# liuyuan-pal/Gen6D

Hardware: NVIDIA H100
Metric: poses/sec end-to-end (128^2 crop, 64 refs, 3 refine iters) (higher is better)
Workload: dtype f32

## Files before the change

### gen6d_b200/_lib.py

```python
import ctypes as C
import os
import re

HERE = os.path.dirname(os.path.abspath(__file__))
LIB_PATH = os.path.join(HERE, 'libgen6d_b200.so')
HEADER_PATH = os.path.join(os.path.dirname(HERE), 'include', 'gen6d_b200.h')

G6D_DET_MAX_SCALES = 8
G6D_GLUE_MAX_OBJECTS = 16
G6D_DET_MAX_INSTANCES = 16
G6D_DET_MAX_PEAK_RADIUS = 3
G6D_DET_MAX_BOXES = 256
G6D_ATTENTION_MAX_SMEM_FLOATS = 12288 - 32
G6D_FRAMES_MAX = 1024
G6D_FRAME_RGB, G6D_FRAME_NV12 = 0, 1
G6D_DRAW_MAX_BOXES = 16
PRO_NONE, PRO_AFFINE, PRO_AFFINE_RELU, PRO_CORR = 0, 1, 2, 3
ACT_NONE, ACT_RELU, ACT_LEAKY01 = 0, 1, 2
TC_TF32, TC_F16 = 0, 1
TC_PRENORM, TC_REUSE_IM2COL, TC_FOLD_SPLITS = 1, 4, 32


class ConvDesc(C.Structure):
    _fields_ = [(n, C.c_int) for n in ('B', 'D', 'H', 'W', 'Cin', 'in_cstride', 'in_coff', 'Cout', 'kd', 'kh', 'kw',
# ... 100 lines not shown
    'g6d_conv_tc_workspace_bytes_ex': [C.POINTER(ConvDesc), I, I],
    'g6d_conv_tc_ex': [C.POINTER(ConvDesc), P, P, P, I, I, P, P, P, P, P, P, L, I, P],
    'g6d_pack_conv_weight_tc': [P, P, P, I, I, I, I, I, P, I, P],
    'g6d_split_operand': [P, P, P, L, I, P],
    'g6d_transpose2d': [P, P, I, I, P],
    'g6d_linear_smallm': [P, P, P, P, I, I, I, I, P],
    'g6d_det_score_fuse': [C.POINTER(DetMaps), I, P, P, P, P, P, P],
    'g6d_det_parse': [P, P, P, I, I, I, I, P, P, P],
    'g6d_det_parse_peaks': [P, P, P, I, I, I, I, I, I, F, F, F, P, P, P, P, P],
    'g6d_det_parse_peaks_host': [P, P, P, I, I, I, I, I, I, F, F, F, P, P, P, P],
    'g6d_det_from_boxes': [P, P, I, I, I, F, P, P, P, P],
    'g6d_det_from_boxes_host': [P, P, I, I, I, F, P, P, P],
    'g6d_det_corr_rowsum': [P, P, I, I, I, I, I, P],
    'g6d_det_corr_rowsum_objects': [P, P, I, I, I, I, I, I, P],
    'g6d_sel_ref_sums': [P, I, I, I, P, P, P],
    'g6d_sel_corr_prologue': [P, P, P, I, I, I, F, P, P, P],
    'g6d_sel_corr_score': [P, P, I, I, I, P, P],
    'g6d_sel_corr_score3': [P, P, P, P, P, P, I, I, I, I, I, P, P, P, P],
    'g6d_sel_corr_score3_workspace_bytes': [I, I, I, I],
    'g6d_sel_vp_norm': [P, I, I, F, P, I, I, P],
    'g6d_sel_max_angle_add': [P, P, P, I, I, I, P],
    'g6d_attention': [P, P, P, P, I, I, I, P],
    'g6d_attention_headmajor': [P, P, P, P, I, I, I, P],
    'g6d_layernorm': [P, P, P, P, I, I, F, P],
    'g6d_sel_parse': [P, P, I, I, P, P, P],
    'g6d_ref_volume_fill': [P, P, P, P, P, P, I, I, I, I, I, I, I, I, P, P, P],
    'g6d_ref_pose_heads': [P, P, P, P, I, I, P],
    'g6d_pose_errors_workspace_bytes': [I, I],
    'g6d_pose_errors': [P, I, P, P, P, I, I, P, P, P],
}
_RESTYPE = {'g6d_pose_errors_workspace_bytes': L, 'g6d_sel_corr_score3_workspace_bytes': L, 'g6d_conv_workspace_bytes': L, 'g6d_conv_tc_workspace_bytes': L, 'g6d_conv_tc_workspace_bytes_ex': L, 'g6d_launch_count': L, 'g6d_last_error': C.c_char_p}

_lib = None


class Gen6DLibraryError(RuntimeError):
    pass

# ... 37 lines not shown
```

### gen6d_b200/csrc/selector.cu

```cuda
#include "common.cuh"

namespace g6d {

template <int C>
__global__ void __launch_bounds__(256) sel_corr_score_kernel(const float* __restrict__ ref,
                                                             const float* __restrict__ q, int S, int P,
                                                             float* __restrict__ score) {
    constexpr int V = C / 128;
    extern __shared__ float t_sh[];
    const int warp = threadIdx.x >> 5, lane = threadIdx.x & 31;
    const int nwarp = blockDim.x >> 5;
    __shared__ float s_red[8];
    for (int s = blockIdx.x; s < S; s += gridDim.x) {
        const float4* rs = reinterpret_cast<const float4*>(ref + (long long)s * P * C);
        float mx = -INFINITY;
        for (int p = warp; p < P; p += nwarp) {
            const float4* rp = rs + (long long)p * (C / 4);
            const float4* qp = reinterpret_cast<const float4*>(q + (long long)p * C);
            float4 rv[V];
#pragma unroll
            for (int i = 0; i < V; ++i) rv[i] = ldg_stream(rp + lane + 32 * i);
            float t = 0.f;
#pragma unroll
            for (int i = 0; i < V; ++i) {
// ... 15 lines not shown
        if (lane == 0) s_red[warp] = acc;
        __syncthreads();
        if (threadIdx.x == 0) {
            float a = 0.f;
            for (int w = 0; w < nwarp; ++w) a += s_red[w];
            score[s] = a;
        }
        __syncthreads();
    }
}

struct ScoreLevels {
    const float* ref[3];
    const float* q[3];
    int P[3];
    int S;
    long long row_end[3];
};

template <int C>
__device__ __forceinline__ float row_dot(const float4* __restrict__ rp, const float4* __restrict__ qp, int lane) {
    constexpr int V = C / 128;
    float4 rv[V];
#pragma unroll
    for (int i = 0; i < V; ++i) rv[i] = ldg_stream(rp + lane + 32 * i);
    float t = 0.f;
#pragma unroll
    for (int i = 0; i < V; ++i) {
        const float4 qv = __ldg(qp + lane + 32 * i);
        t = fmaf(rv[i].x, qv.x, fmaf(rv[i].y, qv.y, fmaf(rv[i].z, qv.z, fmaf(rv[i].w, qv.w, t))));
    }
    return t;
}

template <int C, bool FUSED>
__global__ void __launch_bounds__(256, 6) sel_corr_dots_kernel(const ScoreLevels L, float* __restrict__ t_out,
                                                            int* __restrict__ done, float* __restrict__ score,
                                                            long long chunk) {
    const int lane = threadIdx.x & 31, wib = threadIdx.x >> 5;
    const long long rows = L.row_end[2];
    auto locate = [&](long long row, const float4*& rp, const float4*& qp, int& item, int& P, long long& first) {
        const bool l0 = row < L.row_end[0], l1 = row < L.row_end[1];
        const long long lbase = l0 ? 0 : (l1 ? L.row_end[0] : L.row_end[1]);
        const long long local = row - lbase;
        P = l0 ? L.P[0] : (l1 ? L.P[1] : L.P[2]);
        const float* ref = l0 ? L.ref[0] : (l1 ? L.ref[1] : L.ref[2]);
        const float* q = l0 ? L.q[0] : (l1 ? L.q[1] : L.q[2]);
        const int sl = (int)(local / P);
        const int p = (int)(local - (long long)sl * P);
        item = (l0 ? 0 : (l1 ? 1 : 2)) * L.S + sl;
        first = lbase + (long long)sl * P;
        rp = reinterpret_cast<const float4*>(ref + local * C);
        qp = reinterpret_cast<const float4*>(q + (long long)p * C);
    };
    long long begin, end, stride;
    if (FUSED) {
        begin = (long long)blockIdx.x * chunk;
        end = min(rows, begin + chunk);
        stride = 16;
    } else {
        begin = 0; end = rows;
        stride = (((long long)gridDim.x * blockDim.x) >> 5) * 2;
    }
    const long long w0 = FUSED ? wib : (((long long)blockIdx.x * blockDim.x + threadIdx.x) >> 5);
    for (long long row = begin + w0 * 2; row < end; row += stride) {
        const float4 *r0, *q0, *r1, *q1;
        int item, P;
        long long first;
        locate(row, r0, q0, item, P, first);
        const bool two = row + 1 < end;
        locate(two ? row + 1 : row, r1, q1, item, P, first);
        float t0 = row_dot<C>(r0, q0, lane);
        float t1 = row_dot<C>(r1, q1, lane);
        t0 = warp_sum(t0);
        t1 = warp_sum(t1);
        if (lane == 0) {
            t_out[row] = t0;
            if (two) t_out[row + 1] = t1;
        }
    }
    if (!FUSED) return;
    if (lane == 0) __threadfence();
    __syncthreads();
    int n = 0;
    for (long long r = begin; r < end; ++n) {
        const float4 *rp, *qp;
        int item, P;
        long long first;
        locate(r, rp, qp, item, P, first);
        const long long next = min(end, first + P);
        if ((n & 7) == wib) {
            int last = 0;
            if (lane == 0) last = atomicAdd(done + item, (int)(next - r)) + (int)(next - r) == P;
            last = __shfl_sync(0xffffffffu, last, 0);
            if (last) {
                if (lane == 0) done[item] = 0;
                __threadfence();
                const float* tp = t_out + first;
                float m = -INFINITY;
                for (int p = lane; p < P; p += 32) m = fmaxf(m, __ldcg(tp + p));
                m = warp_max(m);
                float acc = 0.f;
                for (int p = lane; p < P; p += 32) { const float v = __ldcg(tp + p); acc += v * (v / m); }
                acc = warp_sum(acc);
                if (lane == 0) score[item] = acc;
            }
        }
        r = next;
    }
}

__global__ void sel_corr_finish_kernel(const ScoreLevels L, const float* __restrict__ t, float* __restrict__ score) {
    const int lane = threadIdx.x & 31;
    const int item = (int)(((long long)blockIdx.x * blockDim.x + threadIdx.x) >> 5);
    if (item >= 3 * L.S) return;
    const int l = item / L.S, s = item % L.S;
    const int P = l == 0 ? L.P[0] : (l == 1 ? L.P[1] : L.P[2]);
    const float* tp = t + (l == 0 ? 0 : (l == 1 ? L.row_end[0] : L.row_end[1])) + (long long)s * P;
    float m = -INFINITY;
    for (int p = lane; p < P; p += 32) m = fmaxf(m, tp[p]);
    m = warp_max(m);
    float acc = 0.f;
    for (int p = lane; p < P; p += 32) { const float v = tp[p]; acc += v * (v / m); }
    acc = warp_sum(acc);
    if (lane == 0) score[item] = acc;
}

__global__ void sel_ref_sums_kernel(const float* __restrict__ ref, int S, long long PC, int s_chunk,
                                    double* __restrict__ sum1, double* __restrict__ sum2) {
    const long long i = (long long)blockIdx.x * blockDim.x + threadIdx.x;
    if (i >= PC) return;
    const int s0 = blockIdx.y * s_chunk, s1 = min(S, s0 + s_chunk);
    double a = 0.0, b = 0.0;
    for (int s = s0; s < s1; ++s) {
        const double v = (double)ref[(long long)s * PC + i];
        a += v; b += v * v;
    }
    atomicAdd(sum1 + i, a);
    atomicAdd(sum2 + i, b);
}

__global__ void sel_corr_prologue_kernel(const float* __restrict__ q, const double* __restrict__ sum1,
                                         const double* __restrict__ sum2, int S, int P, int C, float eps,
                                         float* __restrict__ scale, float* __restrict__ shift) {
    const int c = blockIdx.x * 32 + (threadIdx.x & 31);
    const int row = threadIdx.x >> 5, nrow = blockDim.x >> 5;
    __shared__ double sm[8][32], sv[8][32];
    __shared__ float s_rstd[32];
    double m = 0.0, e2 = 0.0;
    if (c < C) {
        for (int p = row; p < P; p += nrow) {
            const double qv = (double)q[(long long)p * C + c];
            m += qv * sum1[(long long)p * C + c];
            e2 += qv * qv * sum2[(long long)p * C + c];
        }
    }
    sm[row][threadIdx.x & 31] = m; sv[row][threadIdx.x & 31] = e2;
    __syncthreads();
    if (row == 0 && c < C) {
// ... 3 lines not shown
        double var = e2 / n - mean * mean;
        var = var < 0.0 ? 0.0 : var;
        const double rstd = 1.0 / sqrt(var + (double)eps);
        s_rstd[threadIdx.x] = (float)rstd;
        shift[c] = (float)(-mean * rstd);
    }
    __syncthreads();
    if (c < C) {
        const float r = s_rstd[threadIdx.x & 31];
        for (int p = row; p < P; p += nrow) scale[(long long)p * C + c] = q[(long long)p * C + c] * r;
    }
}

__global__ void sel_vp_norm_kernel(const float* __restrict__ score, int n, float eps, float* __restrict__ feats,
                                   int cstride, int coff) {
    const int l = blockIdx.x;
    const float* s = score + (long long)l * n;
    __shared__ double r1[32], r2[32];
    double a = 0.0, b = 0.0;
    for (int i = threadIdx.x; i < n; i += blockDim.x) { const double v = s[i]; a += v; b += v * v; }
    a = warp_sum(a); b = warp_sum(b);
    if ((threadIdx.x & 31) == 0) { r1[threadIdx.x >> 5] = a; r2[threadIdx.x >> 5] = b; }
    __syncthreads();
    a = 0.0; b = 0.0;
    for (int w = 0; w < (int)(blockDim.x >> 5); ++w) { a += r1[w]; b += r2[w]; }
    const double mean = a / n;
    double var = b / n - mean * mean;
    var = var < 0.0 ? 0.0 : var;
    const float rstd = (float)(1.0 / sqrt(var + (double)eps));
    const float fm = (float)mean;
    for (int i = threadIdx.x; i < n; i += blockDim.x) feats[(long long)i * cstride + coff + l] = (s[i] - fm) * rstd;
    if (l == 0)
        for (int c = coff + (int)gridDim.x; c < cstride; ++c)
            for (int i = threadIdx.x; i < n; i += blockDim.x) feats[(long long)i * cstride + c] = 0.f;
}

__global__ void sel_max_angle_add_kernel(const float* __restrict__ x, const float* __restrict__ embed,
                                         float* __restrict__ out, int rfn, int an, int C) {
    const long long i = (long long)blockIdx.x * blockDim.x + threadIdx.x;
    if (i >= (long long)rfn * C) return;
    const int c = (int)(i % C);
    const int r = (int)(i / C);
    float m = -INFINITY;
    for (int a = 0; a < an; ++a) m = fmaxf(m, x[((long long)r * an + a) * C + c]);
    out[i] = m + embed[i];
}

__global__ void attention_kernel(const float* __restrict__ q, const float* __restrict__ k, const float* __restrict__ v,
                                 float* __restrict__ out, int n, int C, int heads) {
    extern __shared__ float sh[];
    const int i = blockIdx.x, h = blockIdx.y;
    const int D = C / heads;
    float* prob = sh;
// ... 22 lines not shown
    if ((threadIdx.x & 31) == 0) red[threadIdx.x >> 5] = sum;
    __syncthreads();
    sum = 0.f;
    for (int w = 0; w < (int)(blockDim.x >> 5); ++w) sum += red[w];
    for (int d = threadIdx.x; d < D; d += blockDim.x) {
        float acc = 0.f;
        for (int j = 0; j < n; ++j) acc = fmaf(prob[j], v[(long long)j * C + d * heads + h], acc);
        out[(long long)i * C + d * heads + h] = acc / sum;
    }
}

constexpr int ATT_TQ = 8, ATT_TK = 32, ATT_D = 64;
__global__ void __launch_bounds__(128) attention_hm_kernel(const float* __restrict__ q, const float* __restrict__ k,
                                                           const float* __restrict__ v, float* __restrict__ out, int n, int C) {
    extern __shared__ float sh[];
    const int npad = (n + 31) & ~31;
    float* qs = sh;
    float* kt = qs + ATT_TQ * ATT_D;
    float* sc = kt + ATT_TK * (ATT_D + 1);
    __shared__ float s_sum[ATT_TQ];
    const int t = threadIdx.x, lane = t & 31, warp = t >> 5;
    const int i0 = blockIdx.x * ATT_TQ, h = blockIdx.y;
    const float inv = rsqrtf((float)ATT_D);
    for (int e = t; e < ATT_TQ * ATT_D; e += 128) {
        const int qi = e / ATT_D, d = e % ATT_D;
        qs[e] = i0 + qi < n ? q[(long long)(i0 + qi) * C + h * ATT_D + d] : 0.f;
    }
    for (int j0 = 0; j0 < n; j0 += ATT_TK) {
        __syncthreads();
        for (int e = t; e < ATT_TK * ATT_D / 4; e += 128) {
// ... 90 lines not shown
extern "C" int g6d_sel_corr_score(const float* ref, const float* q, int S, int P, int C, float* score,
                                  g6d_stream_t stream) {
    G6D_REQUIRE(ref && q && score && S > 0 && P > 0, "g6d_sel_corr_score: bad args");
    G6D_REQUIRE(C == 512 || C == 256 || C == 128, "g6d_sel_corr_score: C must be 128, 256 or 512 (got %d)", C);
    G6D_REQUIRE(P <= 8192, "g6d_sel_corr_score: P too large");
    const int grid = S < 8 * kNumSMs ? S : 8 * kNumSMs;
    const size_t smem = sizeof(float) * P;
    cudaStream_t st = as_stream(stream);
    if (C == 512) sel_corr_score_kernel<512><<<grid, 256, smem, st>>>(ref, q, S, P, score);
    else if (C == 256) sel_corr_score_kernel<256><<<grid, 256, smem, st>>>(ref, q, S, P, score);
    else sel_corr_score_kernel<128><<<grid, 256, smem, st>>>(ref, q, S, P, score);
    G6D_CHECK_LAUNCH("g6d_sel_corr_score");
    return G6D_OK;
}

extern "C" long long g6d_sel_corr_score3_workspace_bytes(int S, int P0, int P1, int P2) {
    if (S <= 0 || P0 <= 0 || P1 <= 0 || P2 <= 0) { set_error("g6d_sel_corr_score3_workspace_bytes: bad args"); return -1; }
    const long long rows = (long long)S * ((long long)P0 + P1 + P2);
    return ((rows + 3) / 4) * 4 * (long long)sizeof(float);
}

extern "C" int g6d_sel_corr_score3(const float* ref0, const float* ref1, const float* ref2, const float* q0,
                                   const float* q1, const float* q2, int S, int P0, int P1, int P2, int C, float* score,
                                   float* ws, int* counters, g6d_stream_t stream) {
    G6D_REQUIRE(ref0 && ref1 && ref2 && q0 && q1 && q2 && score && ws && S > 0 && P0 > 0 && P1 > 0 && P2 > 0,
                "g6d_sel_corr_score3: bad args");
    G6D_REQUIRE(C == 512, "g6d_sel_corr_score3: C must be 512 (got %d)", C);
    ScoreLevels L;
    L.ref[0] = ref0; L.ref[1] = ref1; L.ref[2] = ref2; L.q[0] = q0; L.q[1] = q1; L.q[2] = q2;
    L.P[0] = P0; L.P[1] = P1; L.P[2] = P2; L.S = S;
    L.row_end[0] = (long long)S * P0; L.row_end[1] = L.row_end[0] + (long long)S * P1;
    L.row_end[2] = L.row_end[1] + (long long)S * P2;
    cudaStream_t st = as_stream(stream);
    static int occ = 0;
    if (occ == 0) {
        int n = 0;
        cudaError_t e = cudaOccupancyMaxActiveBlocksPerMultiprocessor(&n, sel_corr_dots_kernel<512, true>, 256, 0);
        occ = (e == cudaSuccess && n > 0) ? n : 4;
    }
    const long long pairs = (L.row_end[2] + 1) / 2;
    long long grid = (pairs + 7) / 8;
    const long long full = (long long)occ * kNumSMs;
    if (grid > full) grid = full;
    if (counters) {
        int* done = counters;
        long long chunk = (L.row_end[2] + grid - 1) / grid;
        chunk += chunk & 1;
        grid = (L.row_end[2] + chunk - 1) / chunk;
        sel_corr_dots_kernel<512, true><<<(unsigned)grid, 256, 0, st>>>(L, ws, done, score, chunk);
        G6D_CHECK_LAUNCH("g6d_sel_corr_score3");
        return G6D_OK;
    }
    sel_corr_dots_kernel<512, false><<<(unsigned)grid, 256, 0, st>>>(L, ws, nullptr, nullptr, 0);
    G6D_CHECK_LAUNCH("g6d_sel_corr_score3(dots)");
    sel_corr_finish_kernel<<<ceil_div(3ll * S * 32, 256), 256, 0, st>>>(L, ws, score);
    G6D_CHECK_LAUNCH("g6d_sel_corr_score3(finish)");
    return G6D_OK;
}

extern "C" int g6d_sel_ref_sums(const float* ref, int S, int P, int C, double* sum1, double* sum2,
                                g6d_stream_t stream) {
    G6D_REQUIRE(ref && sum1 && sum2 && S > 0 && P > 0 && C > 0, "g6d_sel_ref_sums: bad args");
    const long long PC = (long long)P * C;
    cudaStream_t st = as_stream(stream);
    cudaError_t e = cudaMemsetAsync(sum1, 0, sizeof(double) * PC, st);
    if (e == cudaSuccess) e = cudaMemsetAsync(sum2, 0, sizeof(double) * PC, st);
    if (e != cudaSuccess) { set_error("g6d_sel_ref_sums: memset failed: %s", cudaGetErrorString(e)); return G6D_ECUDA; }
    const int s_chunk = 16;
    dim3 grid(ceil_div(PC, 256), ceil_div(S, s_chunk));
    sel_ref_sums_kernel<<<grid, 256, 0, st>>>(ref, S, PC, s_chunk, sum1, sum2);
    G6D_CHECK_LAUNCH("g6d_sel_ref_sums");
    return G6D_OK;
}

extern "C" int g6d_sel_corr_prologue(const float* q, const double* sum1, const double* sum2, int S, int P, int C,
                                     float eps, float* scale, float* shift, g6d_stream_t stream) {
    G6D_REQUIRE(q && sum1 && sum2 && scale && shift && S > 0 && P > 0 && C > 0, "g6d_sel_corr_prologue: bad args");
    sel_corr_prologue_kernel<<<ceil_div(C, 32), 256, 0, as_stream(stream)>>>(q, sum1, sum2, S, P, C, eps, scale, shift);
    G6D_CHECK_LAUNCH("g6d_sel_corr_prologue");
    return G6D_OK;
}

extern "C" int g6d_sel_vp_norm(const float* score, int L, int n, float eps, float* feats, int cstride, int coff,
                               g6d_stream_t stream) {
    G6D_REQUIRE(score && feats && L > 0 && n > 0 && coff + L <= cstride, "g6d_sel_vp_norm: bad args");
    sel_vp_norm_kernel<<<L, 256, 0, as_stream(stream)>>>(score, n, eps, feats, cstride, coff);
    G6D_CHECK_LAUNCH("g6d_sel_vp_norm");
    return G6D_OK;
}

extern "C" int g6d_sel_max_angle_add(const float* x, const float* embed, float* out, int rfn, int an, int C,
                                     g6d_stream_t stream) {
    G6D_REQUIRE(x && embed && out && rfn > 0 && an > 0 && C > 0, "g6d_sel_max_angle_add: bad args");
    sel_max_angle_add_kernel<<<ceil_div((long long)rfn * C, 256), 256, 0, as_stream(stream)>>>(x, embed, out, rfn, an, C);
    G6D_CHECK_LAUNCH("g6d_sel_max_angle_add");
    return G6D_OK;
}

extern "C" int g6d_attention(const float* q, const float* k, const float* v, float* out, int n, int C, int heads,
                             g6d_stream_t stream) {
    G6D_REQUIRE(q && k && v && out && n > 0 && n <= 8192 && heads > 0 && C % heads == 0, "g6d_attention: bad args");
    G6D_REQUIRE((long long)n + C / heads <= G6D_ATTENTION_MAX_SMEM_FLOATS,
                "g6d_attention: n + C/heads = %lld exceeds the %d floats of shared memory", (long long)n + C / heads,
                G6D_ATTENTION_MAX_SMEM_FLOATS);
    const size_t smem = sizeof(float) * (n + C / heads);
    attention_kernel<<<dim3(n, heads), 64, smem, as_stream(stream)>>>(q, k, v, out, n, C, heads);
    G6D_CHECK_LAUNCH("g6d_attention");
    return G6D_OK;
}

extern "C" int g6d_attention_headmajor(const float* q, const float* k, const float* v, float* out, int n, int C, int heads,
                                       g6d_stream_t stream) {
    G6D_REQUIRE(q && k && v && out && n > 0 && n <= 2048 && heads > 0 && C == heads * ATT_D && (C & 3) == 0,
                "g6d_attention_headmajor: bad args (n <= 2048, C = heads * 64)");
    const int npad = (n + 31) & ~31;
    const size_t smem = sizeof(float) * (ATT_TQ * ATT_D + ATT_TK * (ATT_D + 1) + (size_t)ATT_TQ * npad);
    static bool configured = false;
    if (!configured) {
        cudaError_t e = cudaFuncSetAttribute(attention_hm_kernel, cudaFuncAttributeMaxDynamicSharedMemorySize, 96 * 1024);
        if (e != cudaSuccess) { set_error("g6d_attention_headmajor: %s", cudaGetErrorString(e)); return G6D_ECUDA; }
        configured = true;
    }
    attention_hm_kernel<<<dim3(ceil_div(n, ATT_TQ), heads), 128, smem, as_stream(stream)>>>(q, k, v, out, n, C);
    G6D_CHECK_LAUNCH("g6d_attention_headmajor");
    return G6D_OK;
}

extern "C" int g6d_layernorm(const float* x, const float* gamma, const float* beta, float* out, int rows, int C,
                             float eps, g6d_stream_t stream) {
    G6D_REQUIRE(x && gamma && beta && out && rows > 0 && C > 0, "g6d_layernorm: bad args");
    layernorm_kernel<<<ceil_div(rows, 4), 128, 0, as_stream(stream)>>>(x, gamma, beta, out, rows, C, eps);
    G6D_CHECK_LAUNCH("g6d_layernorm");
    return G6D_OK;
}

extern "C" int g6d_sel_parse(const float* logits, const float* angles, int qn, int rfn, long long* out_idx, float* out,
                             g6d_stream_t stream) {
    G6D_REQUIRE(logits && angles && out_idx && out && qn > 0 && rfn > 0, "g6d_sel_parse: bad args");
    sel_parse_kernel<<<qn, 32, 0, as_stream(stream)>>>(logits, angles, rfn, out_idx, out);
    G6D_CHECK_LAUNCH("g6d_sel_parse");
// ... 3 lines not shown
```

### gen6d_b200/network/selector.py

```python
from dataclasses import dataclass

import numpy as np
import torch

from .. import ops
from .backbone import pack_vgg, vgg_v1
from .base import Branches, PackedModule, linear_as_conv
from .params import SEL_TOWER_POST, SEL_TOWERS, VGG11BNParams, selector_modules

IN_EPS = 1e-5


class LocalComm:
    rank, world, capturable = 0, 1, True

    def all_reduce_sum(self, t):
        return t

    def all_gather_cat(self, t, dim=0):
        return t

    def shard_range(self, n):
        return 0, n

# ... 137 lines not shown
        if i + 1 == len(self.packed()['towers'][level]):
            ops.conv(x, pc, prologue=st['pro'], pro_scale=st['ps'], pro_shift=st['pb'], group_rows=S, out=cat_buf,
                     out_coff=256 * level, plan_rows=rows, **kw)
            return None
        return ops.conv(x, pc, prologue=st['pro'], pro_scale=st['ps'], pro_shift=st['pb'], group_rows=S, stats_rows=rows,
                        plan_rows=rows, **kw) + (rows,)

    @staticmethod
    def _tower_next(st, post, y, ps, pb):
        st['ps'], st['pb'] = ps, pb
        st['pro'] = ops.PRO_AFFINE_RELU if 'r' in post else ops.PRO_AFFINE
        st['x'] = ops.maxpool2x2(y) if 'p' in post else y

    def _tower_state(self, q, ref, s1, s2, S_total):
        Q, h, w, c = q.shape
        pro = [ops.sel_corr_prologue(q[i].reshape(h * w, c), s1, s2, S_total, IN_EPS) for i in range(Q)]
        return {'x': ref, 'ps': [a for a, _ in pro], 'pb': [b for _, b in pro]}

    def _tower(self, level, st, Q, cat_buf, S, refs):
        convs = self.packed()['towers'][level]
        for i, (_, post) in enumerate(convs):
            res = self._tower_conv(level, i, st, Q, S, cat_buf)
            if res is None:
                break
            y, ws, rows = res
            ps, pb = self._finalize(ws, rows // refs.shape[0] * refs.rfn_total)
            self._tower_next(st, post, y, ps, pb)

    def _towers_sharded(self, q_feats, cat_buf, Q, S, S_total, refs):
        towers = self.packed()['towers']
        nbr = 3 if self.comm.capturable else 1
        state = [self._tower_state(q, ref, s1, s2, S_total)
# ... 33 lines not shown
        parts = [self._select_chunk([f[q0:q0 + SEL_QUERY_CHUNK] for f in q_feats], refs, counters)
                 for q0 in range(0, Q, SEL_QUERY_CHUNK)]
        return tuple(torch.cat(t, 0) for t in zip(*parts))

    def _select_chunk(self, q_feats, refs, counters):
        p = self.packed()
        Q = q_feats[0].shape[0]
        rfn, an = refs.shape
        S = rfn * an
        S_total = refs.rfn_total * an
        dev = self.device
        cat_buf = torch.empty(Q * S, 4, 4, 768, device=dev, dtype=torch.float32)
        feats = torch.empty(Q * S, FEAT_PAD, device=dev, dtype=torch.float32)
        scores = torch.empty(Q, 3, S, device=dev, dtype=torch.float32)
        ref_rows = [r.reshape(S, -1, r.shape[-1]) for r in refs.feats_cache]
        for q in range(Q):
            ops.sel_corr_score3(ref_rows, [f[q].reshape(-1, f.shape[-1]) for f in q_feats], counters=counters, out=scores[q])
        if self.comm.world == 1:
            br = Branches(3)
            keep = []

            def one_level(l, q, ref, s1, s2):
                st = self._tower_state(q, ref, s1, s2, S_total)
                keep.append(st)
                self._tower(l, st, Q, cat_buf, S, refs)

            for l, (q, ref, (s1, s2)) in enumerate(zip(q_feats, refs.feats_cache, refs.sums)):
                br.run(l, lambda l=l, q=q, ref=ref, s1=s1, s2=s2: one_level(l, q, ref, s1, s2))
            br.join()
        else:
            self._towers_sharded(q_feats, cat_buf, Q, S, S_total, refs)
        y, ws = ops.conv(cat_buf, p['cf0'], stats_rows=S * 16, plan_rows=S * 16)
        ps, pb = self._finalize(ws, S_total * 16)
        y = ops.avgpool_affine(y.reshape(Q * S * 16, 512), 16, ps, pb, rows_per_group=S * 16, act=ops.ACT_RELU)
        ops.conv(y.reshape(Q * S, 1, 1, 512), p['cf3'], out=feats.reshape(Q * S, 1, 1, FEAT_PAD), out_coff=0, plan_rows=S)
        if self.comm.world == 1:
            for q in range(Q):
                ops.sel_vp_norm(scores[q], feats[q * S:(q + 1) * S], 512, IN_EPS)
        else:
            all_scores = self.comm.all_gather_cat(scores, dim=2).contiguous()
            tmp = torch.empty(Q, S_total, 4, device=dev, dtype=torch.float32)
            for q in range(Q):
                ops.sel_vp_norm(all_scores[q], tmp[q], 0, IN_EPS)
            r0, _ = self.comm.shard_range(refs.rfn_total)
            feats.reshape(Q, S, FEAT_PAD)[:, :, 512:516] = tmp[:, r0 * an:r0 * an + S]
        x = ops.conv(feats.reshape(Q * S, 1, 1, FEAT_PAD), p['sp0'], act=ops.ACT_RELU, plan_rows=S)
        x = ops.conv(x, p['sp2'], plan_rows=S).reshape(Q * rfn, an, 512)
        sf = torch.empty(Q * rfn, 512, device=dev, dtype=torch.float32)
        for q in range(Q):
            ops.sel_max_angle_add(x[q * rfn:(q + 1) * rfn], refs.pose_embed, out=sf[q * rfn:(q + 1) * rfn])
        sf = self.comm.all_gather_cat(sf.reshape(Q, rfn, 512), dim=1).contiguous()
        rfn_local, rfn = rfn, refs.rfn_total
        sf = sf.reshape(Q * rfn, 512)
        for att, (m0, m3) in zip(p['atts'], p['mlps']):
            x4 = sf.reshape(Q * rfn, 1, 1, 512)
            qv = ops.conv(x4, att['conv_query'], plan_rows=rfn).reshape(Q * rfn, 512)
            kv = ops.conv(x4, att['conv_key'], plan_rows=rfn).reshape(Q * rfn, 512)
            vv = ops.conv(x4, att['conv_feats'], plan_rows=rfn).reshape(Q * rfn, 512)
            msg = torch.empty_like(qv)
            for q in range(Q):
                r = slice(q * rfn, (q + 1) * rfn)
                ops.attention(qv[r], kv[r], vv[r], heads=8, head_major=True, out=msg[r])
            msg = ops.conv(msg.reshape(Q * rfn, 1, 1, 512), att['conv_merge'], plan_rows=rfn).reshape(Q * rfn, 512)
            msg = ops.layernorm(msg, att['ln_w'], att['ln_b'], 1e-5)
            y = ops.conv(torch.cat([sf, msg], 1).reshape(Q * rfn, 1, 1, 1024), m0, plan_rows=rfn)
            ps, pb = ops.instnorm_stats(y, rows_per_group=rfn, eps=IN_EPS)
            y = ops.conv(y, m3, prologue=ops.PRO_AFFINE_RELU, pro_scale=ps, pro_shift=pb, group_rows=rfn, plan_rows=rfn)
            ps, pb = ops.instnorm_stats(y, rows_per_group=rfn, eps=IN_EPS)
            y = ops.affine_act(y.reshape(Q * rfn, 512), ps, pb, rows_per_group=rfn, act=ops.ACT_RELU)
            sf = ops.add(y, sf)
        x = ops.conv(sf.reshape(Q * rfn, 1, 1, 512), p['score_predict'][0], act=ops.ACT_RELU, plan_rows=rfn)
        logits = ops.conv(x, p['score_predict'][1], plan_rows=rfn).reshape(Q, rfn)
        x = feats.reshape(Q * rfn_local, 1, 1, an * FEAT_PAD)
        for i, pc in enumerate(p['angle_predict']):
            x = ops.conv(x, pc, act=ops.ACT_RELU if i < 2 else ops.ACT_NONE, plan_rows=rfn_local)
        angles = self.comm.all_gather_cat(x.reshape(Q, rfn_local), dim=1)
        return logits, angles, scores
# ... 87 lines not shown
```

### gen6d_b200/ops.py

```python
import ctypes as C
import os
from dataclasses import dataclass
from typing import Optional

import torch

from . import _lib
from ._lib import ACT_LEAKY01, ACT_NONE, ACT_RELU, PRO_AFFINE, PRO_AFFINE_RELU, PRO_CORR, PRO_NONE


WARP_JOB_BYTES = 88


def _stream():
    return C.c_void_p(torch.cuda.current_stream().cuda_stream)


def _p(t, dtype=torch.float32):
    if t is None:
        return None
    if not (t.is_cuda and t.dtype == dtype and t.is_contiguous()):
        raise ValueError(f'expected a contiguous CUDA {dtype} tensor, got {t.dtype} {t.device} '
                         f'contiguous={t.is_contiguous()} shape={tuple(t.shape)}')
    return C.c_void_p(t.data_ptr())
# ... 731 lines not shown
    count = torch.empty(n, device=dev, dtype=torch.int32)
    _call('g6d_det_from_boxes', _p(boxes), _p(counts, torch.int32), n, N, max_inst, float(inv_box_size), _p(det),
          _p(valid, torch.int32), _p(count, torch.int32), _stream())
    return det, valid, count


def sel_ref_sums(ref):
    S, Pn, Cc = ref.shape
    s1 = torch.empty(Pn, Cc, device=ref.device, dtype=torch.float64)
    s2 = torch.empty_like(s1)
    _call('g6d_sel_ref_sums', _p(ref), S, Pn, Cc, _p(s1, torch.float64), _p(s2, torch.float64), _stream())
    return s1, s2


def sel_corr_prologue(q, s1, s2, S, eps=1e-5):
    Pn, Cc = q.shape
    scale = torch.empty(Pn, Cc, device=q.device, dtype=torch.float32)
    shift = torch.empty(Cc, device=q.device, dtype=torch.float32)
    _call('g6d_sel_corr_prologue', _p(q), _p(s1, torch.float64), _p(s2, torch.float64), S, Pn, Cc, eps, _p(scale),
          _p(shift), _stream())
    return scale, shift


def sel_corr_score(ref, q, out=None):
    S, Pn, Cc = ref.shape
    if out is None:
        out = torch.empty(S, device=ref.device, dtype=torch.float32)
    _call('g6d_sel_corr_score', _p(ref), _p(q), S, Pn, Cc, _p(out), _stream(),
          work=4.0 * (S * Pn * Cc + Pn * Cc + S))
    return out


def sel_corr_score3(refs, qs, counters=None, out=None):
    S, Cc = refs[0].shape[0], refs[0].shape[2]
    Ps = [r.shape[1] for r in refs]
    if out is None:
        out = torch.empty(3, S, device=refs[0].device, dtype=torch.float32)
    ws = torch.empty(_lib.lib().g6d_sel_corr_score3_workspace_bytes(S, *Ps) // 4, device=refs[0].device, dtype=torch.float32)
    _call('g6d_sel_corr_score3', _p(refs[0]), _p(refs[1]), _p(refs[2]), _p(qs[0]), _p(qs[1]), _p(qs[2]), S, Ps[0], Ps[1],
          Ps[2], Cc, _p(out), _p(ws), _p(counters, torch.int32), _stream(), work=4.0 * (S * sum(Ps) * Cc + sum(Ps) * Cc + 3 * S))
    return out


def sel_vp_norm(score, feats, coff, eps=1e-5):
    Ln, n = score.shape
    _call('g6d_sel_vp_norm', _p(score), Ln, n, eps, _p(feats), feats.shape[-1], coff, _stream())


def sel_max_angle_add(x, embed, out=None):
    rfn, an, Cc = x.shape
    if out is None:
        out = torch.empty(rfn, Cc, device=x.device, dtype=torch.float32)
    _call('g6d_sel_max_angle_add', _p(x), _p(embed), _p(out), rfn, an, Cc, _stream())
    return out


def attention(q, k, v, heads, head_major=False, out=None):
    n, Cc = q.shape
    if out is None:
        out = torch.empty_like(q)
    _call('g6d_attention_headmajor' if head_major else 'g6d_attention', _p(q), _p(k), _p(v), _p(out), n, Cc, heads, _stream())
    return out


def layernorm(x, gamma, beta, eps=1e-5):
    rows, Cc = x.shape
    out = torch.empty_like(x)
    _call('g6d_layernorm', _p(x), _p(gamma), _p(beta), _p(out), rows, Cc, eps, _stream())
    return out


def sel_parse(logits, angles):
    qn, rfn = logits.shape
    idx = torch.empty(qn, device=logits.device, dtype=torch.int64)
    out = torch.empty(qn, 2, device=logits.device, dtype=torch.float32)
    _call('g6d_sel_parse', _p(logits), _p(angles), qn, rfn, _p(idx, torch.int64), _p(out), _stream())
# ... 19 lines not shown
```

### include/gen6d_b200.h

```cpp
#ifndef GEN6D_B200_H
#define GEN6D_B200_H

#include <stdint.h>

#ifdef __cplusplus
extern "C" {
#endif

#define G6D_OK 0
#define G6D_EINVAL (-1)
#define G6D_ECUDA (-2)

typedef void* g6d_stream_t;

const char* g6d_last_error(void);
int g6d_version(void);
long long g6d_launch_count(void);

int g6d_preprocess_u8(const uint8_t* img, float* out, long long n_pixels, int out_c, int imagenet_norm,
                      g6d_stream_t stream);
typedef struct g6d_warp_job {
    const uint8_t* src;
    int rows, cols;
    double M[9];
// ... 277 lines not shown
#define G6D_DET_MAX_INSTANCES 16
#define G6D_DET_MAX_PEAK_RADIUS 3
int g6d_det_parse_peaks(const float* scores, const float* scales, const float* offsets, int n_maps, int hs, int ws,
                        int pool_ratio, int max_inst, int radius, float nms_iou, float box_size, float min_score,
                        float* det_out, long long* idx_out, int* valid_out, int* count_out, g6d_stream_t stream);
int g6d_det_parse_peaks_host(const float* scores, const float* scales, const float* offsets, int n_maps, int hs, int ws,
                             int pool_ratio, int max_inst, int radius, float nms_iou, float box_size, float min_score,
                             float* det_out, long long* idx_out, int* valid_out, int* count_out);
#define G6D_DET_MAX_BOXES 256
int g6d_det_from_boxes(const float* boxes, const int* counts, int n_maps, int N, int max_inst, float inv_box_size,
                       float* det_out, int* valid_out, int* count_out, g6d_stream_t stream);
int g6d_det_from_boxes_host(const float* boxes, const int* counts, int n_maps, int N, int max_inst, float inv_box_size,
                            float* det_out, int* valid_out, int* count_out);

int g6d_sel_ref_sums(const float* ref, int S, int P, int C, double* sum1, double* sum2, g6d_stream_t stream);
int g6d_sel_corr_prologue(const float* q, const double* sum1, const double* sum2, int S, int P, int C, float eps,
                          float* scale, float* shift, g6d_stream_t stream);
int g6d_sel_corr_score(const float* ref, const float* q, int S, int P, int C, float* score, g6d_stream_t stream);
long long g6d_sel_corr_score3_workspace_bytes(int S, int P0, int P1, int P2);
int g6d_sel_corr_score3(const float* ref0, const float* ref1, const float* ref2, const float* q0, const float* q1,
                        const float* q2, int S, int P0, int P1, int P2, int C, float* score, float* ws, int* counters,
                        g6d_stream_t stream);
int g6d_sel_vp_norm(const float* score, int L, int n, float eps, float* feats, int cstride, int coff,
                    g6d_stream_t stream);
int g6d_sel_max_angle_add(const float* x, const float* embed, float* out, int rfn, int an, int C, g6d_stream_t stream);
#define G6D_ATTENTION_MAX_SMEM_FLOATS (12288 - 32)
int g6d_attention(const float* q, const float* k, const float* v, float* out, int n, int C, int heads,
                  g6d_stream_t stream);
int g6d_attention_headmajor(const float* q, const float* k, const float* v, float* out, int n, int C, int heads,
                            g6d_stream_t stream);
int g6d_layernorm(const float* x, const float* gamma, const float* beta, float* out, int rows, int C, float eps,
                  g6d_stream_t stream);
int g6d_sel_parse(const float* logits, const float* angles, int qn, int rfn, long long* out_idx, float* out,
                  g6d_stream_t stream);

int g6d_ref_volume_fill(const float* ref_feats, const float* que_feats, const float* ref_Ks,
                        const float* ref_poses, const float* que_Ks, const float* que_poses, int Q, int R,
                        int fh, int fw, int C, int sn, int img_h, int img_w, float* mean_in, float* stdv,
                        g6d_stream_t stream);
int g6d_ref_pose_heads(const float* x, const float* w, const float* b, float* out, int M, int K, g6d_stream_t stream);

long long g6d_pose_errors_workspace_bytes(int n_pts, int n_poses);
int g6d_pose_errors(const float* pts, int n_pts, const float* poses_pr, const float* poses_gt, const float* Ks,
                    int n_poses, int symmetric, float* out, void* ws, g6d_stream_t stream);

// ... 5 lines not shown
```

Baseline: 143.9.

## Batch selector kernels across queries instead of per-query Python loops

Adds a query dimension (Q) to the selector's correlation prologue, corr score, viewpoint norm, max-angle-add and head-major attention kernels. They now use grid.y/z or an inner loop in place of one launch per query. The correlation dots kernel loads each reference row once into registers and reuses it for all queries, cutting repeated ref reads. Launch bounds drop from 6 to 4 blocks per SM to make room for the extra registers, which may lower occupancy.

```diff
diff --git a/gen6d_b200/_lib.py b/gen6d_b200/_lib.py
--- a/gen6d_b200/_lib.py
+++ b/gen6d_b200/_lib.py
@@ -138,14 +138,15 @@
     'g6d_det_corr_rowsum': [P, P, I, I, I, I, I, P],
     'g6d_det_corr_rowsum_objects': [P, P, I, I, I, I, I, I, P],
     'g6d_sel_ref_sums': [P, I, I, I, P, P, P],
-    'g6d_sel_corr_prologue': [P, P, P, I, I, I, F, P, P, P],
+    'g6d_sel_corr_prologue': [P, P, P, I, I, I, I, F, P, P, P],
     'g6d_sel_corr_score': [P, P, I, I, I, P, P],
-    'g6d_sel_corr_score3': [P, P, P, P, P, P, I, I, I, I, I, P, P, P, P],
-    'g6d_sel_corr_score3_workspace_bytes': [I, I, I, I],
-    'g6d_sel_vp_norm': [P, I, I, F, P, I, I, P],
-    'g6d_sel_max_angle_add': [P, P, P, I, I, I, P],
+    'g6d_sel_corr_score3': [P, P, P, P, P, P, I, I, I, I, I, I, P, P, P, P],
+    'g6d_sel_corr_score3_workspace_bytes': [I, I, I, I, I],
+    'g6d_sel_vp_norm': [P, I, I, I, F, P, I, I, P],
+    'g6d_sel_max_angle_add': [P, P, P, I, I, I, I, P],
     'g6d_attention': [P, P, P, P, I, I, I, P],
     'g6d_attention_headmajor': [P, P, P, P, I, I, I, P],
+    'g6d_attention_headmajor_queries': [P, P, P, P, I, I, I, I, P],
     'g6d_layernorm': [P, P, P, P, I, I, F, P],
     'g6d_sel_parse': [P, P, I, I, P, P, P],
     'g6d_ref_volume_fill': [P, P, P, P, P, P, I, I, I, I, I, I, I, I, P, P, P],
diff --git a/gen6d_b200/csrc/selector.cu b/gen6d_b200/csrc/selector.cu
--- a/gen6d_b200/csrc/selector.cu
+++ b/gen6d_b200/csrc/selector.cu
@@ -53,16 +53,13 @@
     const float* ref[3];
     const float* q[3];
     int P[3];
-    int S;
+    int S, nq;
     long long row_end[3];
 };
 
 template <int C>
-__device__ __forceinline__ float row_dot(const float4* __restrict__ rp, const float4* __restrict__ qp, int lane) {
+__device__ __forceinline__ float row_dot(const float4 (&rv)[C / 128], const float4* __restrict__ qp, int lane) {
     constexpr int V = C / 128;
-    float4 rv[V];
-#pragma unroll
-    for (int i = 0; i < V; ++i) rv[i] = ldg_stream(rp + lane + 32 * i);
     float t = 0.f;
 #pragma unroll
     for (int i = 0; i < V; ++i) {
@@ -73,9 +70,10 @@
 }
 
 template <int C, bool FUSED>
-__global__ void __launch_bounds__(256, 6) sel_corr_dots_kernel(const ScoreLevels L, float* __restrict__ t_out,
+__global__ void __launch_bounds__(256, 4) sel_corr_dots_kernel(const ScoreLevels L, float* __restrict__ t_out,
                                                             int* __restrict__ done, float* __restrict__ score,
                                                             long long chunk) {
+    constexpr int V = C / 128;
     const int lane = threadIdx.x & 31, wib = threadIdx.x >> 5;
     const long long rows = L.row_end[2];
     auto locate = [&](long long row, const float4*& rp, const float4*& qp, int& item, int& P, long long& first) {
@@ -104,18 +102,25 @@
     const long long w0 = FUSED ? wib : (((long long)blockIdx.x * blockDim.x + threadIdx.x) >> 5);
     for (long long row = begin + w0 * 2; row < end; row += stride) {
         const float4 *r0, *q0, *r1, *q1;
-        int item, P;
+        int item, P0, P1;
         long long first;
-        locate(row, r0, q0, item, P, first);
+        locate(row, r0, q0, item, P0, first);
         const bool two = row + 1 < end;
-        locate(two ? row + 1 : row, r1, q1, item, P, first);
-        float t0 = row_dot<C>(r0, q0, lane);
-        float t1 = row_dot<C>(r1, q1, lane);
-        t0 = warp_sum(t0);
-        t1 = warp_sum(t1);
-        if (lane == 0) {
-            t_out[row] = t0;
-            if (two) t_out[row + 1] = t1;
+        locate(two ? row + 1 : row, r1, q1, item, P1, first);
+        float4 rv0[V], rv1[V];
+#pragma unroll
+        for (int i = 0; i < V; ++i) rv0[i] = ldg_stream(r0 + lane + 32 * i);
+#pragma unroll
+        for (int i = 0; i < V; ++i) rv1[i] = ldg_stream(r1 + lane + 32 * i);
+        for (int qi = 0; qi < L.nq; ++qi) {
+            float t0 = row_dot<C>(rv0, q0 + (long long)qi * P0 * (C / 4), lane);
+            float t1 = row_dot<C>(rv1, q1 + (long long)qi * P1 * (C / 4), lane);
+            t0 = warp_sum(t0);
+            t1 = warp_sum(t1);
+            if (lane == 0) {
+                t_out[qi * rows + row] = t0;
+                if (two) t_out[qi * rows + row + 1] = t1;
+            }
         }
     }
     if (!FUSED) return;
@@ -135,14 +140,16 @@
             if (last) {
                 if (lane == 0) done[item] = 0;
                 __threadfence();
-                const float* tp = t_out + first;
-                float m = -INFINITY;
-                for (int p = lane; p < P; p += 32) m = fmaxf(m, __ldcg(tp + p));
-                m = warp_max(m);
-                float acc = 0.f;
-                for (int p = lane; p < P; p += 32) { const float v = __ldcg(tp + p); acc += v * (v / m); }
-                acc = warp_sum(acc);
-                if (lane == 0) score[item] = acc;
+                for (int qi = 0; qi < L.nq; ++qi) {
+                    const float* tp = t_out + qi * rows + first;
+                    float m = -INFINITY;
+                    for (int p = lane; p < P; p += 32) m = fmaxf(m, __ldcg(tp + p));
+                    m = warp_max(m);
+                    float acc = 0.f;
+                    for (int p = lane; p < P; p += 32) { const float v = __ldcg(tp + p); acc += v * (v / m); }
+                    acc = warp_sum(acc);
+                    if (lane == 0) score[(long long)qi * 3 * L.S + item] = acc;
+                }
             }
         }
         r = next;
@@ -151,18 +158,19 @@
 
 __global__ void sel_corr_finish_kernel(const ScoreLevels L, const float* __restrict__ t, float* __restrict__ score) {
     const int lane = threadIdx.x & 31;
-    const int item = (int)(((long long)blockIdx.x * blockDim.x + threadIdx.x) >> 5);
-    if (item >= 3 * L.S) return;
+    const long long gi = ((long long)blockIdx.x * blockDim.x + threadIdx.x) >> 5;
+    if (gi >= 3ll * L.S * L.nq) return;
+    const int qi = (int)(gi / (3 * L.S)), item = (int)(gi - (long long)qi * 3 * L.S);
     const int l = item / L.S, s = item % L.S;
     const int P = l == 0 ? L.P[0] : (l == 1 ? L.P[1] : L.P[2]);
-    const float* tp = t + (l == 0 ? 0 : (l == 1 ? L.row_end[0] : L.row_end[1])) + (long long)s * P;
+    const float* tp = t + qi * L.row_end[2] + (l == 0 ? 0 : (l == 1 ? L.row_end[0] : L.row_end[1])) + (long long)s * P;
     float m = -INFINITY;
     for (int p = lane; p < P; p += 32) m = fmaxf(m, tp[p]);
     m = warp_max(m);
     float acc = 0.f;
     for (int p = lane; p < P; p += 32) { const float v = tp[p]; acc += v * (v / m); }
     acc = warp_sum(acc);
-    if (lane == 0) score[item] = acc;
+    if (lane == 0) score[gi] = acc;
 }
 
 __global__ void sel_ref_sums_kernel(const float* __restrict__ ref, int S, long long PC, int s_chunk,
@@ -182,6 +190,9 @@
 __global__ void sel_corr_prologue_kernel(const float* __restrict__ q, const double* __restrict__ sum1,
                                          const double* __restrict__ sum2, int S, int P, int C, float eps,
                                          float* __restrict__ scale, float* __restrict__ shift) {
+    q += (long long)blockIdx.y * P * C;
+    scale += (long long)blockIdx.y * P * C;
+    shift += (long long)blockIdx.y * C;
     const int c = blockIdx.x * 32 + (threadIdx.x & 31);
     const int row = threadIdx.x >> 5, nrow = blockDim.x >> 5;
     __shared__ double sm[8][32], sv[8][32];
@@ -215,6 +226,8 @@
 
 __global__ void sel_vp_norm_kernel(const float* __restrict__ score, int n, float eps, float* __restrict__ feats,
                                    int cstride, int coff) {
+    score += (long long)blockIdx.y * gridDim.x * n;
+    feats += (long long)blockIdx.y * n * cstride;
     const int l = blockIdx.x;
     const float* s = score + (long long)l * n;
     __shared__ double r1[32], r2[32];
@@ -238,6 +251,8 @@
 
 __global__ void sel_max_angle_add_kernel(const float* __restrict__ x, const float* __restrict__ embed,
                                          float* __restrict__ out, int rfn, int an, int C) {
+    x += (long long)blockIdx.y * rfn * an * C;
+    out += (long long)blockIdx.y * rfn * C;
     const long long i = (long long)blockIdx.x * blockDim.x + threadIdx.x;
     if (i >= (long long)rfn * C) return;
     const int c = (int)(i % C);
@@ -290,6 +305,8 @@
 __global__ void __launch_bounds__(128) attention_hm_kernel(const float* __restrict__ q, const float* __restrict__ k,
                                                            const float* __restrict__ v, float* __restrict__ out, int n, int C) {
     extern __shared__ float sh[];
+    const long long qoff = (long long)blockIdx.z * n * C;
+    q += qoff; k += qoff; v += qoff; out += qoff;
     const int npad = (n + 31) & ~31;
     float* qs = sh;
     float* kt = qs + ATT_TQ * ATT_D;
@@ -410,23 +427,24 @@
     return G6D_OK;
 }
 
-extern "C" long long g6d_sel_corr_score3_workspace_bytes(int S, int P0, int P1, int P2) {
-    if (S <= 0 || P0 <= 0 || P1 <= 0 || P2 <= 0) { set_error("g6d_sel_corr_score3_workspace_bytes: bad args"); return -1; }
-    const long long rows = (long long)S * ((long long)P0 + P1 + P2);
+extern "C" long long g6d_sel_corr_score3_workspace_bytes(int S, int P0, int P1, int P2, int Q) {
+    if (S <= 0 || P0 <= 0 || P1 <= 0 || P2 <= 0 || Q <= 0) { set_error("g6d_sel_corr_score3_workspace_bytes: bad args"); return -1; }
+    const long long rows = (long long)Q * S * ((long long)P0 + P1 + P2);
     return ((rows + 3) / 4) * 4 * (long long)sizeof(float);
 }
 
 extern "C" int g6d_sel_corr_score3(const float* ref0, const float* ref1, const float* ref2, const float* q0,
-                                   const float* q1, const float* q2, int S, int P0, int P1, int P2, int C, float* score,
+                                   const float* q1, const float* q2, int S, int P0, int P1, int P2, int C, int Q, float* score,
                                    float* ws, int* counters, g6d_stream_t stream) {
-    G6D_REQUIRE(ref0 && ref1 && ref2 && q0 && q1 && q2 && score && ws && S > 0 && P0 > 0 && P1 > 0 && P2 > 0,
+    G6D_REQUIRE(ref0 && ref1 && ref2 && q0 && q1 && q2 && score && ws && S > 0 && P0 > 0 && P1 > 0 && P2 > 0 && Q > 0,
                 "g6d_sel_corr_score3: bad args");
     G6D_REQUIRE(C == 512, "g6d_sel_corr_score3: C must be 512 (got %d)", C);
     ScoreLevels L;
     L.ref[0] = ref0; L.ref[1] = ref1; L.ref[2] = ref2; L.q[0] = q0; L.q[1] = q1; L.q[2] = q2;
-    L.P[0] = P0; L.P[1] = P1; L.P[2] = P2; L.S = S;
+    L.P[0] = P0; L.P[1] = P1; L.P[2] = P2; L.S = S; L.nq = Q;
     L.row_end[0] = (long long)S * P0; L.row_end[1] = L.row_end[0] + (long long)S * P1;
     L.row_end[2] = L.row_end[1] + (long long)S * P2;
+    G6D_REQUIRE((long long)Q * L.row_end[2] < (1ll << 31), "g6d_sel_corr_score3: Q * S * (P0 + P1 + P2) too large");
     cudaStream_t st = as_stream(stream);
     static int occ = 0;
     if (occ == 0) {
@@ -449,7 +467,7 @@
     }
     sel_corr_dots_kernel<512, false><<<(unsigned)grid, 256, 0, st>>>(L, ws, nullptr, nullptr, 0);
     G6D_CHECK_LAUNCH("g6d_sel_corr_score3(dots)");
-    sel_corr_finish_kernel<<<ceil_div(3ll * S * 32, 256), 256, 0, st>>>(L, ws, score);
+    sel_corr_finish_kernel<<<ceil_div(3ll * S * Q * 32, 256), 256, 0, st>>>(L, ws, score);
     G6D_CHECK_LAUNCH("g6d_sel_corr_score3(finish)");
     return G6D_OK;
 }
@@ -469,26 +487,27 @@
     return G6D_OK;
 }
 
-extern "C" int g6d_sel_corr_prologue(const float* q, const double* sum1, const double* sum2, int S, int P, int C,
+extern "C" int g6d_sel_corr_prologue(const float* q, const double* sum1, const double* sum2, int S, int P, int C, int Q,
                                      float eps, float* scale, float* shift, g6d_stream_t stream) {
-    G6D_REQUIRE(q && sum1 && sum2 && scale && shift && S > 0 && P > 0 && C > 0, "g6d_sel_corr_prologue: bad args");
-    sel_corr_prologue_kernel<<<ceil_div(C, 32), 256, 0, as_stream(stream)>>>(q, sum1, sum2, S, P, C, eps, scale, shift);
+    G6D_REQUIRE(q && sum1 && sum2 && scale && shift && S > 0 && P > 0 && C > 0 && Q > 0 && Q <= 65535,
+                "g6d_sel_corr_prologue: bad args");
+    sel_corr_prologue_kernel<<<dim3(ceil_div(C, 32), Q), 256, 0, as_stream(stream)>>>(q, sum1, sum2, S, P, C, eps, scale, shift);
     G6D_CHECK_LAUNCH("g6d_sel_corr_prologue");
     return G6D_OK;
 }
 
-extern "C" int g6d_sel_vp_norm(const float* score, int L, int n, float eps, float* feats, int cstride, int coff,
+extern "C" int g6d_sel_vp_norm(const float* score, int L, int n, int Q, float eps, float* feats, int cstride, int coff,
                                g6d_stream_t stream) {
-    G6D_REQUIRE(score && feats && L > 0 && n > 0 && coff + L <= cstride, "g6d_sel_vp_norm: bad args");
-    sel_vp_norm_kernel<<<L, 256, 0, as_stream(stream)>>>(score, n, eps, feats, cstride, coff);
+    G6D_REQUIRE(score && feats && L > 0 && n > 0 && Q > 0 && Q <= 65535 && coff + L <= cstride, "g6d_sel_vp_norm: bad args");
+    sel_vp_norm_kernel<<<dim3(L, Q), 256, 0, as_stream(stream)>>>(score, n, eps, feats, cstride, coff);
     G6D_CHECK_LAUNCH("g6d_sel_vp_norm");
     return G6D_OK;
 }
 
-extern "C" int g6d_sel_max_angle_add(const float* x, const float* embed, float* out, int rfn, int an, int C,
+extern "C" int g6d_sel_max_angle_add(const float* x, const float* embed, float* out, int rfn, int an, int C, int Q,
                                      g6d_stream_t stream) {
-    G6D_REQUIRE(x && embed && out && rfn > 0 && an > 0 && C > 0, "g6d_sel_max_angle_add: bad args");
-    sel_max_angle_add_kernel<<<ceil_div((long long)rfn * C, 256), 256, 0, as_stream(stream)>>>(x, embed, out, rfn, an, C);
+    G6D_REQUIRE(x && embed && out && rfn > 0 && an > 0 && C > 0 && Q > 0 && Q <= 65535, "g6d_sel_max_angle_add: bad args");
+    sel_max_angle_add_kernel<<<dim3(ceil_div((long long)rfn * C, 256), Q), 256, 0, as_stream(stream)>>>(x, embed, out, rfn, an, C);
     G6D_CHECK_LAUNCH("g6d_sel_max_angle_add");
     return G6D_OK;
 }
@@ -505,10 +524,10 @@
     return G6D_OK;
 }
 
-extern "C" int g6d_attention_headmajor(const float* q, const float* k, const float* v, float* out, int n, int C, int heads,
-                                       g6d_stream_t stream) {
-    G6D_REQUIRE(q && k && v && out && n > 0 && n <= 2048 && heads > 0 && C == heads * ATT_D && (C & 3) == 0,
-                "g6d_attention_headmajor: bad args (n <= 2048, C = heads * 64)");
+extern "C" int g6d_attention_headmajor_queries(const float* q, const float* k, const float* v, float* out, int n, int C,
+                                               int heads, int Q, g6d_stream_t stream) {
+    G6D_REQUIRE(q && k && v && out && n > 0 && n <= 2048 && heads > 0 && C == heads * ATT_D && (C & 3) == 0 && Q > 0 &&
+                Q <= 65535, "g6d_attention_headmajor: bad args (n <= 2048, C = heads * 64, 0 < Q <= 65535)");
     const int npad = (n + 31) & ~31;
     const size_t smem = sizeof(float) * (ATT_TQ * ATT_D + ATT_TK * (ATT_D + 1) + (size_t)ATT_TQ * npad);
     static bool configured = false;
@@ -517,9 +536,14 @@
         if (e != cudaSuccess) { set_error("g6d_attention_headmajor: %s", cudaGetErrorString(e)); return G6D_ECUDA; }
         configured = true;
     }
-    attention_hm_kernel<<<dim3(ceil_div(n, ATT_TQ), heads), 128, smem, as_stream(stream)>>>(q, k, v, out, n, C);
+    attention_hm_kernel<<<dim3(ceil_div(n, ATT_TQ), heads, Q), 128, smem, as_stream(stream)>>>(q, k, v, out, n, C);
     G6D_CHECK_LAUNCH("g6d_attention_headmajor");
     return G6D_OK;
+}
+
+extern "C" int g6d_attention_headmajor(const float* q, const float* k, const float* v, float* out, int n, int C, int heads,
+                                       g6d_stream_t stream) {
+    return g6d_attention_headmajor_queries(q, k, v, out, n, C, heads, 1, stream);
 }
 
 extern "C" int g6d_layernorm(const float* x, const float* gamma, const float* beta, float* out, int rows, int C,
diff --git a/gen6d_b200/network/selector.py b/gen6d_b200/network/selector.py
--- a/gen6d_b200/network/selector.py
+++ b/gen6d_b200/network/selector.py
@@ -175,8 +175,8 @@
 
     def _tower_state(self, q, ref, s1, s2, S_total):
         Q, h, w, c = q.shape
-        pro = [ops.sel_corr_prologue(q[i].reshape(h * w, c), s1, s2, S_total, IN_EPS) for i in range(Q)]
-        return {'x': ref, 'ps': [a for a, _ in pro], 'pb': [b for _, b in pro]}
+        ps, pb = ops.sel_corr_prologue(q.reshape(Q, h * w, c), s1, s2, S_total, IN_EPS)
+        return {'x': ref, 'ps': ps, 'pb': pb}
 
     def _tower(self, level, st, Q, cat_buf, S, refs):
         convs = self.packed()['towers'][level]
@@ -240,8 +240,7 @@
         feats = torch.empty(Q * S, FEAT_PAD, device=dev, dtype=torch.float32)
         scores = torch.empty(Q, 3, S, device=dev, dtype=torch.float32)
         ref_rows = [r.reshape(S, -1, r.shape[-1]) for r in refs.feats_cache]
-        for q in range(Q):
-            ops.sel_corr_score3(ref_rows, [f[q].reshape(-1, f.shape[-1]) for f in q_feats], counters=counters, out=scores[q])
+        ops.sel_corr_score3(ref_rows, [f.reshape(Q, -1, f.shape[-1]) for f in q_feats], counters=counters, out=scores)
         if self.comm.world == 1:
             br = Branches(3)
             keep = []
@@ -261,20 +260,16 @@
         y = ops.avgpool_affine(y.reshape(Q * S * 16, 512), 16, ps, pb, rows_per_group=S * 16, act=ops.ACT_RELU)
         ops.conv(y.reshape(Q * S, 1, 1, 512), p['cf3'], out=feats.reshape(Q * S, 1, 1, FEAT_PAD), out_coff=0, plan_rows=S)
         if self.comm.world == 1:
-            for q in range(Q):
-                ops.sel_vp_norm(scores[q], feats[q * S:(q + 1) * S], 512, IN_EPS)
+            ops.sel_vp_norm(scores, feats, 512, IN_EPS)
         else:
             all_scores = self.comm.all_gather_cat(scores, dim=2).contiguous()
             tmp = torch.empty(Q, S_total, 4, device=dev, dtype=torch.float32)
-            for q in range(Q):
-                ops.sel_vp_norm(all_scores[q], tmp[q], 0, IN_EPS)
+            ops.sel_vp_norm(all_scores, tmp, 0, IN_EPS)
             r0, _ = self.comm.shard_range(refs.rfn_total)
             feats.reshape(Q, S, FEAT_PAD)[:, :, 512:516] = tmp[:, r0 * an:r0 * an + S]
         x = ops.conv(feats.reshape(Q * S, 1, 1, FEAT_PAD), p['sp0'], act=ops.ACT_RELU, plan_rows=S)
         x = ops.conv(x, p['sp2'], plan_rows=S).reshape(Q * rfn, an, 512)
-        sf = torch.empty(Q * rfn, 512, device=dev, dtype=torch.float32)
-        for q in range(Q):
-            ops.sel_max_angle_add(x[q * rfn:(q + 1) * rfn], refs.pose_embed, out=sf[q * rfn:(q + 1) * rfn])
+        sf = ops.sel_max_angle_add(x, refs.pose_embed)
         sf = self.comm.all_gather_cat(sf.reshape(Q, rfn, 512), dim=1).contiguous()
         rfn_local, rfn = rfn, refs.rfn_total
         sf = sf.reshape(Q * rfn, 512)
@@ -283,10 +278,7 @@
             qv = ops.conv(x4, att['conv_query'], plan_rows=rfn).reshape(Q * rfn, 512)
             kv = ops.conv(x4, att['conv_key'], plan_rows=rfn).reshape(Q * rfn, 512)
             vv = ops.conv(x4, att['conv_feats'], plan_rows=rfn).reshape(Q * rfn, 512)
-            msg = torch.empty_like(qv)
-            for q in range(Q):
-                r = slice(q * rfn, (q + 1) * rfn)
-                ops.attention(qv[r], kv[r], vv[r], heads=8, head_major=True, out=msg[r])
+            msg = ops.attention(*(t.reshape(Q, rfn, 512) for t in (qv, kv, vv)), heads=8, head_major=True)
             msg = ops.conv(msg.reshape(Q * rfn, 1, 1, 512), att['conv_merge'], plan_rows=rfn).reshape(Q * rfn, 512)
             msg = ops.layernorm(msg, att['ln_w'], att['ln_b'], 1e-5)
             y = ops.conv(torch.cat([sf, msg], 1).reshape(Q * rfn, 1, 1, 1024), m0, plan_rows=rfn)
diff --git a/gen6d_b200/ops.py b/gen6d_b200/ops.py
--- a/gen6d_b200/ops.py
+++ b/gen6d_b200/ops.py
@@ -769,10 +769,11 @@
 
 
 def sel_corr_prologue(q, s1, s2, S, eps=1e-5):
-    Pn, Cc = q.shape
-    scale = torch.empty(Pn, Cc, device=q.device, dtype=torch.float32)
-    shift = torch.empty(Cc, device=q.device, dtype=torch.float32)
-    _call('g6d_sel_corr_prologue', _p(q), _p(s1, torch.float64), _p(s2, torch.float64), S, Pn, Cc, eps, _p(scale),
+    Pn, Cc = q.shape[-2:]
+    Q = q.shape[0] if q.dim() == 3 else 1
+    scale = torch.empty(q.shape, device=q.device, dtype=torch.float32)
+    shift = torch.empty(q.shape[:-2] + (Cc,), device=q.device, dtype=torch.float32)
+    _call('g6d_sel_corr_prologue', _p(q), _p(s1, torch.float64), _p(s2, torch.float64), S, Pn, Cc, Q, eps, _p(scale),
           _p(shift), _stream())
     return scale, shift
 
@@ -789,32 +790,44 @@
 def sel_corr_score3(refs, qs, counters=None, out=None):
     S, Cc = refs[0].shape[0], refs[0].shape[2]
     Ps = [r.shape[1] for r in refs]
+    Q = qs[0].shape[0] if qs[0].dim() == 3 else 1
     if out is None:
-        out = torch.empty(3, S, device=refs[0].device, dtype=torch.float32)
-    ws = torch.empty(_lib.lib().g6d_sel_corr_score3_workspace_bytes(S, *Ps) // 4, device=refs[0].device, dtype=torch.float32)
+        out = torch.empty(qs[0].shape[:-2] + (3, S), device=refs[0].device, dtype=torch.float32)
+    ws = torch.empty(_lib.lib().g6d_sel_corr_score3_workspace_bytes(S, *Ps, Q) // 4, device=refs[0].device, dtype=torch.float32)
     _call('g6d_sel_corr_score3', _p(refs[0]), _p(refs[1]), _p(refs[2]), _p(qs[0]), _p(qs[1]), _p(qs[2]), S, Ps[0], Ps[1],
-          Ps[2], Cc, _p(out), _p(ws), _p(counters, torch.int32), _stream(), work=4.0 * (S * sum(Ps) * Cc + sum(Ps) * Cc + 3 * S))
+          Ps[2], Cc, Q, _p(out), _p(ws), _p(counters, torch.int32), _stream(),
+          work=4.0 * (S * sum(Ps) * Cc + Q * sum(Ps) * Cc + 3 * Q * S))
     return out
 
 
 def sel_vp_norm(score, feats, coff, eps=1e-5):
-    Ln, n = score.shape
-    _call('g6d_sel_vp_norm', _p(score), Ln, n, eps, _p(feats), feats.shape[-1], coff, _stream())
+    Ln, n = score.shape[-2:]
+    Q = score.shape[0] if score.dim() == 3 else 1
+    _call('g6d_sel_vp_norm', _p(score), Ln, n, Q, eps, _p(feats), feats.shape[-1], coff, _stream())
 
 
 def sel_max_angle_add(x, embed, out=None):
-    rfn, an, Cc = x.shape
+    rows, an, Cc = x.shape
+    rfn = embed.shape[0]
+    if rows % rfn:
+        raise ValueError(f'sel_max_angle_add: {rows} rows are not whole queries of {rfn} references')
     if out is None:
-        out = torch.empty(rfn, Cc, device=x.device, dtype=torch.float32)
-    _call('g6d_sel_max_angle_add', _p(x), _p(embed), _p(out), rfn, an, Cc, _stream())
+        out = torch.empty(rows, Cc, device=x.device, dtype=torch.float32)
+    _call('g6d_sel_max_angle_add', _p(x), _p(embed), _p(out), rfn, an, Cc, rows // rfn, _stream())
     return out
 
 
 def attention(q, k, v, heads, head_major=False, out=None):
-    n, Cc = q.shape
+    n, Cc = q.shape[-2:]
     if out is None:
         out = torch.empty_like(q)
-    _call('g6d_attention_headmajor' if head_major else 'g6d_attention', _p(q), _p(k), _p(v), _p(out), n, Cc, heads, _stream())
+    if head_major:
+        Q = q.shape[0] if q.dim() == 3 else 1
+        _call('g6d_attention_headmajor_queries', _p(q), _p(k), _p(v), _p(out), n, Cc, heads, Q, _stream())
+    else:
+        if q.dim() != 2:
+            raise ValueError('attention: the reference channel order takes one [n, C] problem per call')
+        _call('g6d_attention', _p(q), _p(k), _p(v), _p(out), n, Cc, heads, _stream())
     return out
 
 
diff --git a/include/gen6d_b200.h b/include/gen6d_b200.h
--- a/include/gen6d_b200.h
+++ b/include/gen6d_b200.h
@@ -315,21 +315,24 @@
                             float* det_out, int* valid_out, int* count_out);
 
 int g6d_sel_ref_sums(const float* ref, int S, int P, int C, double* sum1, double* sum2, g6d_stream_t stream);
-int g6d_sel_corr_prologue(const float* q, const double* sum1, const double* sum2, int S, int P, int C, float eps,
+int g6d_sel_corr_prologue(const float* q, const double* sum1, const double* sum2, int S, int P, int C, int Q, float eps,
                           float* scale, float* shift, g6d_stream_t stream);
 int g6d_sel_corr_score(const float* ref, const float* q, int S, int P, int C, float* score, g6d_stream_t stream);
-long long g6d_sel_corr_score3_workspace_bytes(int S, int P0, int P1, int P2);
+long long g6d_sel_corr_score3_workspace_bytes(int S, int P0, int P1, int P2, int Q);
 int g6d_sel_corr_score3(const float* ref0, const float* ref1, const float* ref2, const float* q0, const float* q1,
-                        const float* q2, int S, int P0, int P1, int P2, int C, float* score, float* ws, int* counters,
-                        g6d_stream_t stream);
-int g6d_sel_vp_norm(const float* score, int L, int n, float eps, float* feats, int cstride, int coff,
+                        const float* q2, int S, int P0, int P1, int P2, int C, int Q, float* score, float* ws,
+                        int* counters, g6d_stream_t stream);
+int g6d_sel_vp_norm(const float* score, int L, int n, int Q, float eps, float* feats, int cstride, int coff,
                     g6d_stream_t stream);
-int g6d_sel_max_angle_add(const float* x, const float* embed, float* out, int rfn, int an, int C, g6d_stream_t stream);
+int g6d_sel_max_angle_add(const float* x, const float* embed, float* out, int rfn, int an, int C, int Q,
+                          g6d_stream_t stream);
 #define G6D_ATTENTION_MAX_SMEM_FLOATS (12288 - 32)
 int g6d_attention(const float* q, const float* k, const float* v, float* out, int n, int C, int heads,
                   g6d_stream_t stream);
 int g6d_attention_headmajor(const float* q, const float* k, const float* v, float* out, int n, int C, int heads,
                             g6d_stream_t stream);
+int g6d_attention_headmajor_queries(const float* q, const float* k, const float* v, float* out, int n, int C, int heads,
+                                    int Q, g6d_stream_t stream);
 int g6d_layernorm(const float* x, const float* gamma, const float* beta, float* out, int rows, int C, float eps,
                   g6d_stream_t stream);
 int g6d_sel_parse(const float* logits, const float* angles, int qn, int rfn, long long* out_idx, float* out,
```

New measurement: 144.1 (median of 6 runs). Within noise of the previous version (+0.1%).
